# lambdaclass/noir_backend_using_gnark

Hardware: AMD Instinct MI355X
Metric: Groth16 prove ms + BN254 G1 MSM scalar-muls/sec at 2^20 / 2^24 constraints (higher is better)
Workload: dtype u32

## Files before the change

### noir_backend_using_gnark_amd/csrc/groth16.hip

```cpp
#include <stdlib.h>
#include <chrono>
#include <functional>
#include <memory>
#include <vector>
#include <string.h>

#include "ctx.hpp"
#include "curve.hpp"
#include "host_ff.hpp"
#include "keyio.hpp"
#include "msm.hpp"
#include "multidev.hpp"
#include "ntt.hpp"
#include "proofio.hpp"

namespace zkmi {

template <class F>
struct FixedBase {
    std::vector<XYZZ<F>> tab;
    void build(const Affine<F>& p) {
        tab.resize(32 * 256);
        XYZZ<F> base = XYZZ<F>::from_affine(p);
        for (int w = 0; w < 32; w++) {
// ... 320 lines not shown
    auto it = g_pks.find(handle);
    if (it == g_pks.end()) return set_err(ZK_ERR_HANDLE, "unknown proving-key handle %llu", (unsigned long long)handle);
    if (n_wires) *n_wires = it->second.n_wires;
    if (n_public) *n_public = it->second.n_public;
    if (log_domain) *log_domain = it->second.log_domain;
    if (has_tables) *has_tables = it->second.tables ? 1 : 0;
    return ZK_OK;
}

struct Msm5Inputs {
    const void *d_a, *d_b, *d_b2, *d_w;
    size_t nw;
    const void *d_k, *d_wk;
    size_t nk;
    const void *d_z, *d_h;
    size_t nz;
    const MsmTable *tab_w = nullptr, *tab_h = nullptr;
    const void *t_a = nullptr, *t_b = nullptr, *t_b2 = nullptr, *t_k = nullptr, *t_z = nullptr;
};
static const zk_msm_cfg kMontCfg = {0, 1, 0, 0};

static bool k_shares_w(const Msm5Inputs& in, size_t* j) {
    if (!in.nk || !in.nw) return false;
    ptrdiff_t d = (const char*)in.d_wk - (const char*)in.d_w;
    if (d < 0 || d % 32) return false;
    *j = (size_t)d / 32;
    return *j + in.nk == in.nw;
}

struct Msm5State {
    MsmJob jobs[5];
    MsmPrep prep_w, prep_h;
    hipStream_t chain = nullptr;
};

static int msm5_prepare_w(Slot* sl[5], const Msm5Inputs& in, hipEvent_t ev_w, Msm5State* S) {
    static const bool low = ZK_EXP("ZKMI_PREPW_LOW", 0) == 1;
    hipStream_t st4 = low ? sl[4]->stream : sl[4]->hi();
    if (ev_w) ZK_HIP(hipStreamWaitEvent(st4, ev_w, 0));
    static const bool drop = ZK_EXP("ZKMI_W_DROP_ZERO_DIGITS", 1) != 0;
    if (in.tab_w) return msm_prepare_scalars_table(sl[4], st4, in.d_w, in.nw, &kMontCfg, *in.tab_w, &S->prep_w, drop);
    return msm_prepare_scalars(sl[4], st4, in.d_w, in.nw, &kMontCfg, &S->prep_w, drop);
}
typedef std::function<int(hipEvent_t g2_done, hipEvent_t* gate_next)> BetweenFn;
static int msm5_accumulate_w(Slot* sl[5], const Msm5Inputs& in, hipEvent_t ev_w, Msm5State* S, hipEvent_t gate_first_acc, const BetweenFn* between = nullptr);
static int msm5_launch_w(Slot* sl[5], const Msm5Inputs& in, hipEvent_t ev_w, Msm5State* S, hipEvent_t gate_first_acc = nullptr) {
    ZK_TRY(msm5_prepare_w(sl, in, ev_w, S));
    return msm5_accumulate_w(sl, in, ev_w, S, gate_first_acc);
}
static int msm5_accumulate_w(Slot* sl[5], const Msm5Inputs& in, hipEvent_t ev_w, Msm5State* S, hipEvent_t gate_first_acc, const BetweenFn* between) {
    hipStream_t st4 = sl[4]->hi();
    size_t j = 0;
    const bool share_k = k_shares_w(in, &j);
    static const bool one_chain = ZK_EXP("ZKMI_CHAIN", 0) == 1;
    if (one_chain && (in.tab_w || share_k)) {
        hipStream_t chain = sl[4]->stream;
        S->jobs[4].gate_acc = gate_first_acc;
        S->jobs[4].chain = chain;
        ZK_TRY(msm_g2_accumulate(sl[4], st4, S->prep_w, in.tab_w ? in.t_b2 : in.d_b2, 0, &S->jobs[4]));
        S->jobs[1].chain = chain;
        ZK_TRY(msm_g1_accumulate(sl[1], sl[1]->stream, S->prep_w, in.tab_w ? in.t_a : in.d_a, 0, &S->jobs[1]));
        S->jobs[2].chain = chain;
        ZK_TRY(msm_g1_accumulate(sl[2], sl[2]->stream, S->prep_w, in.tab_w ? in.t_b : in.d_b, 0, &S->jobs[2]));
        S->jobs[3].chain = chain;
        S->jobs[3].want_done = true;
        if (in.tab_w) ZK_TRY(msm_g1_accumulate(sl[3], sl[3]->stream, S->prep_w, in.t_k, 0, &S->jobs[3]));
        else ZK_TRY(msm_g1_accumulate(sl[3], sl[3]->stream, S->prep_w, (const char*)in.d_k - j * 64, (uint32_t)j, &S->jobs[3]));
        return ZK_OK;
    }
    S->jobs[4].gate_acc = gate_first_acc;
    S->jobs[4].want_done = true;
    ZK_TRY(msm_g2_accumulate(sl[4], st4, S->prep_w, in.tab_w ? in.t_b2 : in.d_b2, 0, &S->jobs[4]));
    hipEvent_t prev = S->jobs[4].acc_done;
    if (between) ZK_TRY((*between)(S->jobs[4].acc_done, &prev));
    static const bool batch_acc = ZK_EXP("ZKMI_BATCH_ACC", 0) == 1;
    if (batch_acc && (in.tab_w || share_k)) {
        Slot* bs[3] = {sl[1], sl[2], sl[3]};
        hipStream_t bst[3] = {sl[1]->stream, sl[2]->stream, sl[3]->stream};
        const void* bp[3] = {in.tab_w ? in.t_a : in.d_a, in.tab_w ? in.t_b : in.d_b, in.tab_w ? in.t_k : (const void*)((const char*)in.d_k - j * 64)};
        uint32_t bskip[3] = {0, 0, in.tab_w ? 0u : (uint32_t)j};
        MsmJob* bj[3] = {&S->jobs[1], &S->jobs[2], &S->jobs[3]};
        S->jobs[1].gate_acc = prev;
        S->jobs[3].want_done = true;
        return msm_g1_accumulate_batch(3, bs, bst, S->prep_w, bp, bskip, bj);
    }
    S->jobs[1].gate_acc = prev;
    S->jobs[1].want_done = true;
    ZK_TRY(msm_g1_accumulate(sl[1], sl[1]->stream, S->prep_w, in.tab_w ? in.t_a : in.d_a, 0, &S->jobs[1]));
    if (S->jobs[1].acc_done) prev = S->jobs[1].acc_done;
    S->jobs[2].gate_acc = prev;
    S->jobs[2].want_done = true;
    ZK_TRY(msm_g1_accumulate(sl[2], sl[2]->stream, S->prep_w, in.tab_w ? in.t_b : in.d_b, 0, &S->jobs[2]));
    if (S->jobs[2].acc_done) prev = S->jobs[2].acc_done;
    S->jobs[3].gate_acc = prev;
    S->jobs[3].want_done = true;
    if (in.tab_w) {
        ZK_TRY(msm_g1_accumulate(sl[3], sl[3]->stream, S->prep_w, in.t_k, 0, &S->jobs[3]));
    } else if (share_k) {
        ZK_TRY(msm_g1_accumulate(sl[3], sl[3]->stream, S->prep_w, (const char*)in.d_k - j * 64, (uint32_t)j, &S->jobs[3]));
    } else {
        if (ev_w) ZK_HIP(hipStreamWaitEvent(sl[3]->stream, ev_w, 0));
        ZK_TRY(msm_g1_launch(sl[3], sl[3]->stream, in.d_k, in.d_wk, in.nk, &kMontCfg, &S->jobs[3]));
    }
    return ZK_OK;
}
static int msm5_prepare_h(Slot* sl[5], hipStream_t st0, const Msm5Inputs& in, Msm5State* S) {
    if (in.tab_h) return msm_prepare_scalars_table(sl[0], st0, in.d_h, in.nz, &kMontCfg, *in.tab_h, &S->prep_h);
    return msm_prepare_scalars(sl[0], st0, in.d_h, in.nz, &kMontCfg, &S->prep_h);
}
static int msm5_launch_h(Slot* sl[5], hipStream_t st0, const Msm5Inputs& in, Msm5State* S, bool prepared = false) {
    static const bool preph_low = ZK_EXP("ZKMI_PREPH_LOW", 0) == 1;
    if (!prepared && preph_low && sl[0]->stream != st0) {
        hipEvent_t ev;
        ZK_HIP(hipEventCreateWithFlags(&ev, hipEventDisableTiming));
        ZK_HIP(hipEventRecord(ev, st0));
        ZK_HIP(hipStreamWaitEvent(sl[0]->stream, ev, 0));
        (void)hipEventDestroy(ev);
        ZK_TRY(msm5_prepare_h(sl, sl[0]->stream, in, S));
        prepared = true;
    }
    if (!prepared) ZK_TRY(msm5_prepare_h(sl, st0, in, S));
    S->jobs[0].chain = S->chain;
    if (!S->chain) {
        hipEvent_t prev = nullptr;
        for (int i : {4, 1, 2, 3})
            if (S->jobs[i].acc_done) prev = S->jobs[i].acc_done;
        S->jobs[0].gate_acc = prev;
    }
    static const bool quad_tail = ZK_EXP("ZKMI_QUAD_TAIL", 0) == 1;
    S->jobs[0].quad_tail = quad_tail;
    ZK_TRY(msm_g1_accumulate(sl[0], st0, S->prep_h, in.tab_h ? in.t_z : in.d_z, 0, &S->jobs[0]));
    return ZK_OK;
}
static int msm5_finish(Msm5State* S, uint64_t out[96], const std::function<void(const XYZZ<HFp>&, const XYZZ<HFp>&)>* early = nullptr) {
    XYZZ<HFp> m_a, m_b, m_k, m_z;
    XYZZ<HFp2> m_b2;
    int rc = msm_g2_finish(S->jobs[4], &m_b2);
    if (rc == ZK_OK) rc = msm_g1_finish(S->jobs[1], &m_a);
    if (rc == ZK_OK) rc = msm_g1_finish(S->jobs[2], &m_b);
    if (rc == ZK_OK && early) (*early)(m_a, m_b);
    if (rc == ZK_OK) rc = msm_g1_finish(S->jobs[3], &m_k);
    if (rc == ZK_OK) rc = msm_g1_finish(S->jobs[0], &m_z);
    msm_prep_release(&S->prep_w);
    msm_prep_release(&S->prep_h);
    for (int i = 0; i < 5; i++)
        if (S->jobs[i].acc_done) { (void)hipEventDestroy(S->jobs[i].acc_done); S->jobs[i].acc_done = nullptr; }
    ZK_TRY(rc);
    memcpy(out, &m_a, 128);
    memcpy(out + 16, &m_b, 128);
    memcpy(out + 32, &m_k, 128);
    memcpy(out + 48, &m_z, 128);
    memcpy(out + 64, &m_b2, 256);
    return ZK_OK;
}
static int msm5_reserve(Slot* sl[5], const Msm5Inputs& in, size_t extra0) {
    size_t need[5] = {0, 0, 0, 0, 0}, prep = 0, acc1 = 0, acc2 = 0, j = 0;
    if (in.tab_h) {
        size_t ph = 0, ah = 0;
        ZK_TRY(msm_prep_need_table(in.nz, *in.tab_h, sl[0]->stream, &ph, &ah, nullptr));
        need[0] = ph + ah;
    } else {
        ZK_TRY(msm_g1_need(in.nz, &kMontCfg, sl[0]->stream, &need[0]));
    }
// ... 290 lines not shown
        in.t_a = P.t_a; in.t_b = P.t_b; in.t_b2 = P.t_b2; in.t_k = P.t_k; in.t_z = P.t_z;
    }
    ZK_TRY(msm5_reserve(g.s, in, 3 * N * 32 + nw * 32 + 4096));
    hipMemcpyKind kind = on_device ? hipMemcpyDeviceToDevice : hipMemcpyHostToDevice;
    hipStream_t st4 = g.s[4]->hi();
    int rc = ZK_OK;
    Fr* d_abc[3] = {nullptr, nullptr, nullptr};
    const void* src[3] = {a, b, c};
    const bool direct = on_device && n_constraints == N && N > 1;
    static const bool host_order_on = (ZK_EXP("ZKMI_HOST_ORDER", 1) != 0);
    const bool host_order = !on_device && host_order_on && nw > 0 && N > 1;
    Fr* d_w = (Fr*)s0->alloc(nw * 32 + 16);
    for (int i = 0; i < 3; i++) d_abc[i] = (Fr*)s0->alloc(N * 32);
    if (on_device) d_w = (Fr*)const_cast<void*>(w);
    auto upload_abc = [&]() -> int {
        for (int i = 0; i < 3; i++) {
            if (direct) continue;
            if (n_constraints && hipMemcpyAsync(d_abc[i], src[i], n_constraints * 32, kind, st) != hipSuccess) return set_err(ZK_ERR_HIP, "hipMemcpyAsync failed");
            if (n_constraints < N && hipMemsetAsync(d_abc[i] + n_constraints, 0, (N - n_constraints) * 32, st) != hipSuccess) return set_err(ZK_ERR_HIP, "hipMemsetAsync failed");
        }
        return ZK_OK;
    };
    const Fr* in_place_src[3] = {(const Fr*)a, (const Fr*)b, (const Fr*)c};
    static const bool h_streams = ZK_EXP("ZKMI_H_STREAMS", 0) == 1;
    const hipStream_t side[2] = {g.s[1]->hi(), g.s[2]->hi()};
    hipEvent_t ev_h = nullptr;
    auto run_compute_h = [&]() -> int {
        ZK_TRY(compute_h_inplace(s0, st, d_abc[0], d_abc[1], d_abc[2], P.log_domain, direct ? in_place_src : nullptr, h_streams ? side : nullptr));
        ZK_HIP(hipEventCreateWithFlags(&ev_h, hipEventDisableTiming));
        ZK_HIP(hipEventRecord(ev_h, st));
        return ZK_OK;
    };
    Msm5State S;
    static const bool nogate = ZK_EXP("ZKMI_NOGATE", 0) == 1;
    static const bool preph_first = ZK_EXP("ZKMI_PREPH_FIRST", 0) == 1;
    static const bool preph_early = ZK_EXP("ZKMI_PREPH_EARLY", 0) == 1;
    if (host_order) {
        if (hipMemcpyAsync(d_w, w, nw * 32, kind, st4) != hipSuccess) rc = set_err(ZK_ERR_HIP, "hipMemcpyAsync failed");
        in.d_w = d_w;
        in.d_wk = d_w + P.n_public;
        in.d_h = d_abc[0];
        if (rc == ZK_OK) rc = msm5_prepare_w(g.s, in, nullptr, &S);
        if (rc == ZK_OK) rc = upload_abc();
        const BetweenFn between = [&](hipEvent_t g2_done, hipEvent_t* gate_next) -> int {
            if (g2_done) ZK_HIP(hipStreamWaitEvent(st, g2_done, 0));
            ZK_TRY(run_compute_h());
            *gate_next = ev_h;
            return ZK_OK;
        };
        if (rc == ZK_OK) rc = msm5_accumulate_w(g.s, in, nullptr, &S, nullptr, &between);
        if (rc == ZK_OK) rc = msm5_launch_h(g.s, st, in, &S);
    } else {
        static const bool h_under_g2 = ZK_EXP("ZKMI_H_UNDER_G2", 0) == 1;
        if (h_under_g2) {
            if (!on_device && nw && hipMemcpyAsync(d_w, w, nw * 32, kind, st4) != hipSuccess) rc = set_err(ZK_ERR_HIP, "hipMemcpyAsync failed");
            in.d_w = d_w;
            in.d_wk = d_w + P.n_public;
            in.d_h = d_abc[0];
            if (rc == ZK_OK) rc = msm5_prepare_w(g.s, in, nullptr, &S);
            if (rc == ZK_OK) rc = upload_abc();
            if (rc == ZK_OK && S.prep_w.ready && hipStreamWaitEvent(st, S.prep_w.ready, 0) != hipSuccess) rc = set_err(ZK_ERR_HIP, "hipStreamWaitEvent failed");
            if (rc == ZK_OK) rc = run_compute_h();
            if (rc == ZK_OK) rc = msm5_accumulate_w(g.s, in, nullptr, &S, nullptr);
            if (rc == ZK_OK) rc = msm5_launch_h(g.s, st, in, &S);
        } else {
        rc = upload_abc();
// ... 39 lines not shown
```

### noir_backend_using_gnark_amd/csrc/msm.hip

```cpp
#include <math.h>
#include <string.h>

#include <algorithm>
#include <memory>
#include <tuple>
#include <type_traits>

#ifdef ZKMI_EXPERIMENTS
#include "experiments/msm_rocprim_include.inc"
#endif

#include <chrono>
#include "ctx.hpp"
#include "curve.hpp"
#include "ff29.hpp"
#include "host_ff.hpp"
#include "msm.hpp"
#include "multidev.hpp"
#include "radix.hpp"

namespace zkmi {

struct PingPong {
    uint32_t* b[2];
// ... 685 lines not shown
            for (uint32_t t = t0 + lane; t < t1; t += 64) acc.add(TailPt<F>::load(partial + t));
        }
        const uint32_t cnt = min(nheld, 64u);
        unsigned first = 32;
        while (first >= cnt && first > 0) first >>= 1;
        for (unsigned d = first; d > 0; d >>= 1) {
            TailPt<F> o = acc.shfl_down(d);
            if (lane < d) acc.add(o);
        }
        if (lane == 0) acc.store(partial + t0);
    }
}

template <class F, class PT = TailPt<F>>
__global__ __launch_bounds__(256) void k_reduce_l1(const XYZZ<F>* __restrict__ partial, const uint32_t* __restrict__ task_off, uint32_t B,
                                                   uint32_t W, uint32_t m, XYZZ<F>* __restrict__ A_out, XYZZ<F>* __restrict__ S_out) {
    prio_hi();
    uint32_t N1 = B / m;
    uint32_t g = (blockIdx.x * blockDim.x + threadIdx.x) / PT::LPP;
    if (g >= W * N1) return;
    uint32_t w = g / N1, q = g % N1;
    uint32_t b0 = w * B + q * m;
    PT run = PT::inf(), acc = PT::inf();
    for (int l = (int)m - 1; l >= 0; l--) {
        uint32_t b = b0 + l;
        uint32_t t0 = task_off[b];
        if (task_off[b + 1] > t0) run.add(PT::load(partial + t0));
        acc.add(run);
    }
    if (threadIdx.x % PT::LPP == 0) {
        acc.store(A_out + g);
        run.store(S_out + g);
    }
}

template <class F>
__global__ __launch_bounds__(256) void k_reduce_l2(const XYZZ<F>* __restrict__ A_in, const XYZZ<F>* __restrict__ S_in, uint32_t N, uint32_t W, uint32_t sh,
                                                   uint32_t m, XYZZ<F>* __restrict__ A_out, XYZZ<F>* __restrict__ S_out) {
    prio_hi();
    typedef TailPt<F> PT;
    uint32_t Nout = (N + m - 1) / m;
    uint32_t g = blockIdx.x * blockDim.x + threadIdx.x;
    if (g >= W * Nout) return;
    uint32_t w = g / Nout, q = g % Nout;
    PT run = PT::inf(), t = PT::inf(), asum = PT::inf();
    for (int l = (int)m - 1; l >= 0; l--) {
        uint32_t j = q * m + (uint32_t)l;
        if (j >= N) continue;
        asum.add(PT::load(A_in + (size_t)w * N + j));
        run.add(PT::load(S_in + (size_t)w * N + j));
        if (l >= 1) t.add(run);
    }
    for (uint32_t i = 0; i < sh; i++) t.dbl();
    asum.add(t);
    asum.store(A_out + g);
    run.store(S_out + g);
}

template <class F, class PT = TailPt<F>>
__global__ __launch_bounds__(64) void k_reduce_wave(const XYZZ<F>* __restrict__ A_in, const XYZZ<F>* __restrict__ S_in, uint32_t N, uint32_t W,
                                                    uint32_t sh, XYZZ<F>* __restrict__ A_out, XYZZ<F>* __restrict__ S_out) {
    prio_hi();
    constexpr uint32_t FAN = 64 / PT::LPP;
    uint32_t Nout = (N + FAN - 1) / FAN;
    uint32_t chunk = blockIdx.x;
    uint32_t w = chunk / Nout, q = chunk % Nout;
// ... 226 lines not shown
#include "experiments/msm_scan_rocprim_call.inc"
#endif
    if (own_scan) ZK_TRY(xs_exclusive_scan(s, st, scan_tmp, ntasks, task_off, (size_t)nb + 1));
    }
    uint32_t bshift = 0;
    while ((L >> bshift) >= TS_BINS) bshift++;
    const uint32_t nbins = (L >> bshift) + 1;
    const unsigned tgrid = (unsigned)((max_tasks + 255) / 256);
    static const bool merged_fill = ZK_EXP("ZKMI_PREP_MERGE", 1) == 2;
    if (merged_fill) {
        ZK_LAUNCH(s, st, "msm_task_fill", k_task_fill_bins, dim3(tgrid), dim3(256), 0, (const uint32_t*)start, (const uint32_t*)task_off, nb, L, bins, (uint32_t)max_tasks, bshift,
                  nbins, task_begin, lkey0, hist);
    } else {
        ZK_LAUNCH(s, st, "msm_task_fill", k_task_fill, dim3(tgrid), dim3(256), 0, (const uint32_t*)start, (const uint32_t*)task_off, nb, L, (const uint32_t*)bins,
                  (uint32_t)max_tasks, bshift, nbins, task_begin, lkey0, hist);
        ZK_LAUNCH(s, st, "msm_task_bins", k_task_bins, dim3(1), dim3(256), 0, hist, nbins);
    }
    ZK_LAUNCH(s, st, "msm_task_scatter", k_task_scatter, dim3(tgrid), dim3(256), 0, (const uint32_t*)lkey0, (uint32_t)max_tasks, bshift, nbins, hist,
              lkey1, tid1);
    out->vals = vb.current();
    out->start = start;
    out->task_off = task_off;
    out->task_begin = task_begin;
    out->lkeys = lkey1;
    out->tids = tid1;
    out->multi_list = multi_list;
    out->num_multi = num_multi;
    ZK_HIP(hipEventCreateWithFlags(&out->ready, hipEventDisableTiming));
    ZK_HIP(hipEventRecord(out->ready, st));
    return ZK_OK;
}

template <class F>
static int msm_accumulate_batch(int nb, Slot* const* sl, const hipStream_t* sts, const MsmPrep& R, const void* const* d_pts, const uint32_t* skip_below,
                                MsmJob* const* jobs) {
    typedef XYZZ<F> Pt;
    const MsmPlan& P = R.P;
    for (int b = 0; b < nb; b++) {
        jobs[b]->s = sl[b];
        jobs[b]->st = sts[b];
        jobs[b]->c = P.c;
        jobs[b]->W = P.W;
        jobs[b]->empty = R.empty;
    }
    if (R.empty) return ZK_OK;
    const unsigned W = P.W;
    const uint32_t B = P.B, L = P.L, m1 = P.m1, N1 = P.N1;
    const size_t max_tasks = P.max_tasks, lvl_elems = P.lvl_elems;
    Pt *partial[3], *lvlA[3][2], *lvlS[3][2];
    AccBatch batch = {};
    for (int b = 0; b < nb; b++) {
        Slot* s = sl[b];
        partial[b] = (Pt*)s->alloc(max_tasks * sizeof(Pt));
        for (int k = 0; k < 2; k++) {
            lvlA[b][k] = (Pt*)s->alloc((lvl_elems + 64) * sizeof(Pt));
            lvlS[b][k] = (Pt*)s->alloc((lvl_elems + 64) * sizeof(Pt));
        }
        if (!partial[b] || !lvlA[b][0] || !lvlA[b][1] || !lvlS[b][0] || !lvlS[b][1])
            return set_err(ZK_ERR_HIP, "MSM workspace was not reserved up front (%zu bytes needed)", P.need_acc);
        batch.pts[b] = d_pts[b];
        batch.partial[b] = partial[b];
        batch.skip_below[b] = skip_below[b];
    }
    MsmJob* j0 = jobs[0];
    hipStream_t sa = j0->chain ? j0->chain : sts[0];
    if (R.ready) ZK_HIP(hipStreamWaitEvent(sa, R.ready, 0));
// ... 39 lines not shown
        }
    }
#endif
    if (!launched) ZK_LAUNCH(sl[0], sa, acc_name, (k_accumulate<F>), dim3(full_grid, (unsigned)nb), dim3(256), acc_shmem, batch, R.vals, R.task_begin, R.lkeys, R.tids, L, (uint32_t)max_tasks);
    if (T) {
        hipEvent_t& e = T->ring[T->next];
        if (!e) ZK_HIP(hipEventCreateWithFlags(&e, hipEventDisableTiming));
        ZK_HIP(hipEventRecord(e, sa));
        T->last = e;
        T->next = (T->next + 1) % 16;
        turn_lock.unlock();
    }
    bool want = j0->chain != nullptr || nb > 1;
    for (int b = 0; b < nb; b++) want = want || jobs[b]->want_done;
    if (want) {
        hipEvent_t done;
        ZK_HIP(hipEventCreateWithFlags(&done, hipEventDisableTiming));
        ZK_HIP(hipEventRecord(done, sa));
        jobs[nb - 1]->acc_done = done;
        for (int b = 0; b < nb; b++)
            if (sts[b] != sa) ZK_HIP(hipStreamWaitEvent(sts[b], done, 0));
    }
    for (int b = 0; b < nb; b++) {
        Slot* s = sl[b];
        hipStream_t st = sts[b];
        bool folded = false;
#ifdef ZKMI_EXPERIMENTS
#include "experiments/msm_tail_fused_launch.inc"
#endif
        if (!folded) {
            ZK_LAUNCH(s, st, "msm_fold_giant", (k_fold_giant<F>), dim3(GIANT_MAX * 16), dim3(256), 0, partial[b], R.task_off, (const uint32_t*)R.num_multi);
            ZK_LAUNCH(s, st, "msm_fold_multi", (k_fold_multi<F>), dim3(1024), dim3(256), 0, partial[b], R.task_off, R.multi_list, R.num_multi);
        }
        bool quad = false;
        if constexpr (sizeof(F) == sizeof(Fp)) quad = jobs[b]->quad_tail;
        const uint32_t lpp = quad ? 4 : 1, fan = 64 / lpp, fan_log = quad ? 4 : 6;
        ZK_LAUNCH(s, st, "msm_reduce_l1", (k_reduce_l1<F>), dim3((unsigned)(((size_t)W * N1 + 255) / 256)), dim3(256), 0, (const Pt*)partial[b], R.task_off, B, W,
                  m1, lvlA[b][0], lvlS[b][0]);
        uint32_t N = N1, sh = 0;
        for (uint32_t mm = m1; mm > 1; mm >>= 1) sh++;
        int cur = 0;
        if (P.m2 > 1 && N > 64 * P.m2) {
            uint32_t Nout = (N + P.m2 - 1) / P.m2;
            ZK_LAUNCH(s, st, "msm_reduce_l2", (k_reduce_l2<F>), dim3((unsigned)(((size_t)W * Nout + 255) / 256)), dim3(256), 0, (const Pt*)lvlA[b][cur],
                      (const Pt*)lvlS[b][cur], N, W, sh, P.m2, lvlA[b][cur ^ 1], lvlS[b][cur ^ 1]);
            cur ^= 1;
            N = Nout;
            for (uint32_t mm = P.m2; mm > 1; mm >>= 1) sh++;
        }
        const uint32_t host_n = (W * 64 <= 64) ? 64 : 1;
        while (N > host_n) {
            uint32_t Nout = (N + fan - 1) / fan;
            if constexpr (sizeof(F) == sizeof(Fp)) {
                if (quad) ZK_LAUNCH(s, st, "msm_reduce_wave", (k_reduce_wave<F, TailPtQ>), dim3(W * Nout), dim3(64), 0, (const Pt*)lvlA[b][cur], (const Pt*)lvlS[b][cur], N, W, sh, lvlA[b][cur ^ 1], lvlS[b][cur ^ 1]);
            }
            if (!quad) ZK_LAUNCH(s, st, "msm_reduce_wave", (k_reduce_wave<F>), dim3(W * Nout), dim3(64), 0, (const Pt*)lvlA[b][cur], (const Pt*)lvlS[b][cur], N, W, sh, lvlA[b][cur ^ 1], lvlS[b][cur ^ 1]);
            cur ^= 1;
            N = Nout;
            sh += fan_log;
        }
        jobs[b]->n_final = N;
        jobs[b]->sh_final = sh;
        const size_t cnt = (size_t)W * N;
        ZK_TRY(s->pinned_reserve(2 * cnt * sizeof(Pt)));
        ZK_HIP(hipMemcpyAsync(s->pinned, lvlA[b][cur], cnt * sizeof(Pt), hipMemcpyDeviceToHost, st));
        if (N > 1) ZK_HIP(hipMemcpyAsync((char*)s->pinned + cnt * sizeof(Pt), lvlS[b][cur], cnt * sizeof(Pt), hipMemcpyDeviceToHost, st));
    }
    return ZK_OK;
}

template <class F>
static int msm_accumulate(Slot* s, hipStream_t st, const MsmPrep& R, const Affine<F>* d_pts, uint32_t skip_below, MsmJob* job) {
    const void* pts = d_pts;
    return msm_accumulate_batch<F>(1, &s, &st, R, &pts, &skip_below, &job);
}

template <class F>
static int msm_launch(Slot* s, hipStream_t st, const MsmPlan& P, const Affine<F>* d_pts, const Fr* d_scalars, size_t n, const zk_msm_cfg* cfg,
                      MsmJob* job) {
    MsmPrep R;
    ZK_TRY(msm_prepare(s, st, P, d_scalars, n, cfg, &R));
    int rc = msm_accumulate<F>(s, st, R, d_pts, 0, job);
    if (R.ready) (void)hipEventDestroy(R.ready);
    return rc;
}

template <class HF>
static int msm_finish(const MsmJob& job, XYZZ<HF>* total_out, XYZZ<HF>* per_set = nullptr) {
    *total_out = XYZZ<HF>::inf();
    if (per_set)
        for (unsigned w = 0; w < (job.empty ? 3u : job.W); w++) per_set[w] = XYZZ<HF>::inf();
    if (job.empty) return ZK_OK;
    ZK_TRY(slot_sync(job.s, job.st));
    const unsigned N = job.n_final;
    if constexpr (sizeof(HF) == sizeof(HFp)) {
        static const HFp inv32 = HFp{{32, 0, 0, 0}}.to_mont().inv();
        XYZZ<HFp>* w = reinterpret_cast<XYZZ<HFp>*>(job.s->pinned);
        const size_t cnt = (size_t)job.W * N * (N > 1 ? 2 : 1);
        for (size_t i = 0; i < cnt; i++) {
            w[i].x = w[i].x * inv32;
            w[i].y = w[i].y * inv32;
            w[i].zz = w[i].zz * inv32;
            w[i].zzz = w[i].zzz * inv32;
        }
    }
    const XYZZ<HF>* wa = reinterpret_cast<const XYZZ<HF>*>(job.s->pinned);
    const XYZZ<HF>* wsum = wa + (size_t)job.W * N;
// ... 176 lines not shown
    uint32_t j = src_idx[i];
    Affine<F> p;
    uint4* d = reinterpret_cast<uint4*>(&p);
    if (j == 0xffffffffu) {
#pragma unroll
        for (unsigned k = 0; k < sizeof(p) / 16; k++) d[k] = make_uint4(0, 0, 0, 0);
    } else {
        p = gload(compact + j);
    }
    gstore(out + i, p);
}
int msm_expand_bases(Slot* s, hipStream_t st, int is_g2, const void* d_compact, const uint32_t* d_src_idx, size_t n, void* d_out) {
    if (!n) return ZK_OK;
    if (is_g2)
        ZK_LAUNCH(s, st, "pk_expand_bases_g2", (k_expand_bases<Fp2>), dim3((unsigned)((n + 255) / 256)), dim3(256), 0, (const Affine<Fp2>*)d_compact, d_src_idx,
                  (uint32_t)n, (Affine<Fp2>*)d_out);
    else
        ZK_LAUNCH(s, st, "pk_expand_bases_g1", (k_expand_bases<Fp>), dim3((unsigned)((n + 255) / 256)), dim3(256), 0, (const Affine<Fp>*)d_compact, d_src_idx,
                  (uint32_t)n, (Affine<Fp>*)d_out);
    return ZK_OK;
}

int msm_prepare_scalars(Slot* s, hipStream_t st, const void* d_scalars, size_t n, const zk_msm_cfg* cfg, MsmPrep* out, bool drop_zero_digits) {
    MsmPlan P;
    ZK_TRY(msm_plan<Fp>(n, cfg, st, &P));
    return msm_prepare(s, st, P, (const Fr*)d_scalars, n, cfg, out, nullptr, drop_zero_digits);
}
void msm_prep_release(MsmPrep* R) {
    if (R->ready) (void)hipEventDestroy(R->ready);
    R->ready = nullptr;
}
int msm_g1_accumulate(Slot* s, hipStream_t st, const MsmPrep& R, const void* d_pts, uint32_t skip_below, MsmJob* job) {
    return msm_accumulate<Fp>(s, st, R, (const Affine<Fp>*)d_pts, skip_below, job);
}
int msm_g1_accumulate_batch(int nb, Slot* const* sl, const hipStream_t* sts, const MsmPrep& R, const void* const* d_pts, const uint32_t* skip_below,
                            MsmJob* const* jobs) {
    if (nb < 1 || nb > 3) return set_err(ZK_ERR_ARG, "accumulate batch of %d", nb);
    return msm_accumulate_batch<Fp>(nb, sl, sts, R, d_pts, skip_below, jobs);
}
int msm_g2_accumulate(Slot* s, hipStream_t st, const MsmPrep& R, const void* d_pts, uint32_t skip_below, MsmJob* job) {
    return msm_accumulate<Fp2>(s, st, R, (const Affine<Fp2>*)d_pts, skip_below, job);
}
int msm_g1_finish(const MsmJob& job, XYZZ<HFp>* out) { return msm_finish<HFp>(job, out); }
int msm_g1_finish_batch(const MsmJob& job, XYZZ<HFp> out[3]) {
    XYZZ<HFp> unused;
    return msm_finish<HFp>(job, &unused, out);
}
int msm_g2_finish(const MsmJob& job, XYZZ<HFp2>* out) { return msm_finish<HFp2>(job, out); }
int msm_g1_xyzz(Slot* s, hipStream_t st, const void* d_pts, const void* d_scalars, size_t n, const zk_msm_cfg* cfg, XYZZ<HFp>* out) {
    MsmJob job;
    ZK_TRY(msm_g1_launch(s, st, d_pts, d_scalars, n, cfg, &job));
    return msm_g1_finish(job, out);
}
int msm_g2_xyzz(Slot* s, hipStream_t st, const void* d_pts, const void* d_scalars, size_t n, const zk_msm_cfg* cfg, XYZZ<HFp2>* out) {
    MsmJob job;
    ZK_TRY(msm_g2_launch(s, st, d_pts, d_scalars, n, cfg, &job));
    return msm_g2_finish(job, out);
}

static int check_cfg(const zk_msm_cfg* cfg) {
    if (cfg && cfg->nb_tasks > 1024) return set_err(ZK_ERR_NB_TASKS, "invalid config: config.NbTasks > 1024");
    return ZK_OK;
}

struct Bases {
    void* d = nullptr;
// ... 569 lines not shown
```

### noir_backend_using_gnark_amd/csrc/msm.hpp

```cpp
#pragma once
#include "ctx.hpp"
#include "curve.hpp"
#include "host_ff.hpp"

namespace zkmi {

unsigned msm_pick_window(size_t n);
int msm_g1_need(size_t n, const zk_msm_cfg* cfg, hipStream_t st, size_t* need);
int msm_g2_need(size_t n, const zk_msm_cfg* cfg, hipStream_t st, size_t* need);
struct MsmTable {
    unsigned c = 0;
    size_t stride = 0;
    unsigned row_first = 0, row_step = 1;
    unsigned rows() const {
        unsigned Wd = (255 + c - 1) / c;
        return row_first < Wd ? (Wd - 1 - row_first) / row_step + 1 : 0;
    }
    unsigned l2_m = 0;
    unsigned l1_m = 0;
};
unsigned msm_pick_window_table(size_t n);
int msm_build_table_g1(Slot* s, hipStream_t st, const void* d_pts, size_t n, size_t stride, size_t offset, unsigned c, void* d_table, unsigned row_first = 0,
                       unsigned row_step = 1);
int msm_build_table_g2(Slot* s, hipStream_t st, const void* d_pts, size_t n, size_t stride, size_t offset, unsigned c, void* d_table, unsigned row_first = 0,
// ... 22 lines not shown
    hipEvent_t ready = nullptr;
};

struct MsmJob {
    Slot* s = nullptr;
    hipStream_t st = nullptr;
    unsigned c = 0, W = 0;
    unsigned n_final = 1, sh_final = 0;
    bool empty = true;
    hipEvent_t gate_acc = nullptr;
    bool want_done = false;
    hipEvent_t acc_done = nullptr;
    hipStream_t chain = nullptr;
    bool turnstile = false;
    bool quad_tail = false;
};
int msm_g1_launch(Slot* s, hipStream_t st, const void* d_pts, const void* d_scalars, size_t n, const zk_msm_cfg* cfg, MsmJob* job);
int msm_g2_launch(Slot* s, hipStream_t st, const void* d_pts, const void* d_scalars, size_t n, const zk_msm_cfg* cfg, MsmJob* job);
int msm_prep_need(size_t n, const zk_msm_cfg* cfg, hipStream_t st, size_t* need_prep, size_t* need_acc_g1, size_t* need_acc_g2);
int msm_prepare_scalars(Slot* s, hipStream_t st, const void* d_scalars, size_t n, const zk_msm_cfg* cfg, MsmPrep* out, bool drop_zero_digits = false);
int msm_prep_need_table(size_t n, const MsmTable& tab, hipStream_t st, size_t* need_prep, size_t* need_acc_g1, size_t* need_acc_g2);
int msm_prepare_scalars_table(Slot* s, hipStream_t st, const void* d_scalars, size_t n, const zk_msm_cfg* cfg, const MsmTable& tab, MsmPrep* out, bool drop_zero_digits = false);
int msm_prep_need_table_batch(size_t n, unsigned sets, const MsmTable& tab, hipStream_t st, size_t* need_prep, size_t* need_acc_g1);
int msm_prepare_scalars_table_batch(Slot* s, hipStream_t st, const void* const* d_scalars, unsigned sets, size_t n, const zk_msm_cfg* cfg, const MsmTable& tab, MsmPrep* out,
                                    bool drop_zero_digits = false);
size_t msm_compact_need(size_t n, unsigned sets);
int msm_bases_batch_dev_sparse(uint64_t handle, size_t offset, const void* const* d_scalars, unsigned count, size_t n, const zk_msm_cfg* cfg, void* out);
int msm_g1_finish_batch(const MsmJob& job, XYZZ<HFp> out[3]);
void msm_prep_release(MsmPrep* R);
int msm_g1_accumulate(Slot* s, hipStream_t st, const MsmPrep& R, const void* d_pts, uint32_t skip_below, MsmJob* job);
int msm_g2_accumulate(Slot* s, hipStream_t st, const MsmPrep& R, const void* d_pts, uint32_t skip_below, MsmJob* job);
int msm_g1_accumulate_batch(int nb, Slot* const* sl, const hipStream_t* sts, const MsmPrep& R, const void* const* d_pts, const uint32_t* skip_below,
                            MsmJob* const* jobs);
int msm_g1_finish(const MsmJob& job, XYZZ<HFp>* out);
int msm_g2_finish(const MsmJob& job, XYZZ<HFp2>* out);
int msm_g1_xyzz(Slot* s, hipStream_t st, const void* d_pts, const void* d_scalars, size_t n, const zk_msm_cfg* cfg, XYZZ<HFp>* out);
int msm_g2_xyzz(Slot* s, hipStream_t st, const void* d_pts, const void* d_scalars, size_t n, const zk_msm_cfg* cfg, XYZZ<HFp2>* out);

}
```

Measured before the change: 449.6 million.

## Merge K and H MSMs into one shared bucket reduction tail

When the witness K MSM and the H/Z MSM use the same bucket layout, both are still accumulated into their own per-task partials. A new pair kernel then sums the two bucket sets inside a single level-1 reduction, so only one reduction chain and one host finish run instead of two. The reduction code is moved into a shared helper to support this. It adds cross-stream event dependencies and skips the separate K job, which relies on the finish step treating that job as empty.

```diff
diff --git a/noir_backend_using_gnark_amd/csrc/groth16.hip b/noir_backend_using_gnark_amd/csrc/groth16.hip
--- a/noir_backend_using_gnark_amd/csrc/groth16.hip
+++ b/noir_backend_using_gnark_amd/csrc/groth16.hip
@@ -376,7 +376,18 @@
     MsmJob jobs[5];
     MsmPrep prep_w, prep_h;
     hipStream_t chain = nullptr;
+    bool kz_allowed = false, kz = false;
 };
+
+static bool kz_merge(const Msm5Inputs& in, hipStream_t st) {
+    static const bool on = ZK_EXP("ZKMI_KZ_MERGE", 1) != 0;
+    size_t j = 0;
+    if (!on || !in.nw || !in.nk || !in.nz || (in.tab_w == nullptr) != (in.tab_h == nullptr)) return false;
+    if (in.tab_w && (in.tab_w->row_step > 1 || in.tab_h->row_step > 1)) return false;
+    if (!in.tab_w && !k_shares_w(in, &j)) return false;
+    bool ok = false;
+    return msm_g1_pair_ok(in.nw, in.tab_w, in.nz, in.tab_h, &kMontCfg, st, &ok) == ZK_OK && ok;
+}
 
 static int msm5_prepare_w(Slot* sl[5], const Msm5Inputs& in, hipEvent_t ev_w, Msm5State* S) {
     static const bool low = ZK_EXP("ZKMI_PREPW_LOW", 0) == 1;
@@ -396,8 +407,10 @@
     hipStream_t st4 = sl[4]->hi();
     size_t j = 0;
     const bool share_k = k_shares_w(in, &j);
+    S->kz = S->kz_allowed && kz_merge(in, st4);
     static const bool one_chain = ZK_EXP("ZKMI_CHAIN", 0) == 1;
     if (one_chain && (in.tab_w || share_k)) {
+        S->kz = false;
         hipStream_t chain = sl[4]->stream;
         S->jobs[4].gate_acc = gate_first_acc;
         S->jobs[4].chain = chain;
@@ -419,6 +432,7 @@
     if (between) ZK_TRY((*between)(S->jobs[4].acc_done, &prev));
     static const bool batch_acc = ZK_EXP("ZKMI_BATCH_ACC", 0) == 1;
     if (batch_acc && (in.tab_w || share_k)) {
+        S->kz = false;
         Slot* bs[3] = {sl[1], sl[2], sl[3]};
         hipStream_t bst[3] = {sl[1]->stream, sl[2]->stream, sl[3]->stream};
         const void* bp[3] = {in.tab_w ? in.t_a : in.d_a, in.tab_w ? in.t_b : in.d_b, in.tab_w ? in.t_k : (const void*)((const char*)in.d_k - j * 64)};
@@ -435,6 +449,7 @@
     S->jobs[2].gate_acc = prev;
     S->jobs[2].want_done = true;
     ZK_TRY(msm_g1_accumulate(sl[2], sl[2]->stream, S->prep_w, in.tab_w ? in.t_b : in.d_b, 0, &S->jobs[2]));
+    if (S->kz) return ZK_OK;
     if (S->jobs[2].acc_done) prev = S->jobs[2].acc_done;
     S->jobs[3].gate_acc = prev;
     S->jobs[3].want_done = true;
@@ -473,6 +488,16 @@
     }
     static const bool quad_tail = ZK_EXP("ZKMI_QUAD_TAIL", 0) == 1;
     S->jobs[0].quad_tail = quad_tail;
+    if (S->kz) {
+        size_t j = 0;
+        const bool share_k = !in.tab_w && k_shares_w(in, &j);
+        Slot* const psl[2] = {sl[3], sl[0]};
+        const hipStream_t psts[2] = {sl[3]->stream, st0};
+        const MsmPrep* const pR[2] = {&S->prep_w, &S->prep_h};
+        const void* const ppts[2] = {in.tab_w ? in.t_k : (const void*)((const char*)in.d_k - j * 64), in.tab_h ? in.t_z : in.d_z};
+        const uint32_t pskip[2] = {share_k ? (uint32_t)j : 0u, 0u};
+        return msm_g1_accumulate_pair(psl, psts, pR, ppts, pskip, &S->jobs[0]);
+    }
     ZK_TRY(msm_g1_accumulate(sl[0], st0, S->prep_h, in.tab_h ? in.t_z : in.d_z, 0, &S->jobs[0]));
     return ZK_OK;
 }
@@ -829,6 +854,7 @@
         return ZK_OK;
     };
     Msm5State S;
+    S.kz_allowed = true;
     static const bool nogate = ZK_EXP("ZKMI_NOGATE", 0) == 1;
     static const bool preph_first = ZK_EXP("ZKMI_PREPH_FIRST", 0) == 1;
     static const bool preph_early = ZK_EXP("ZKMI_PREPH_EARLY", 0) == 1;
diff --git a/noir_backend_using_gnark_amd/csrc/msm.hip b/noir_backend_using_gnark_amd/csrc/msm.hip
--- a/noir_backend_using_gnark_amd/csrc/msm.hip
+++ b/noir_backend_using_gnark_amd/csrc/msm.hip
@@ -741,6 +741,28 @@
         acc.store(A_out + g);
         run.store(S_out + g);
     }
+}
+template <class F>
+__global__ __launch_bounds__(256) void k_reduce_l1_pair(const XYZZ<F>* __restrict__ partial0, const uint32_t* __restrict__ task_off0,
+                                                        const XYZZ<F>* __restrict__ partial1, const uint32_t* __restrict__ task_off1, uint32_t B, uint32_t W,
+                                                        uint32_t m, XYZZ<F>* __restrict__ A_out, XYZZ<F>* __restrict__ S_out) {
+    prio_hi();
+    typedef TailPt<F> PT;
+    uint32_t N1 = B / m;
+    uint32_t g = blockIdx.x * blockDim.x + threadIdx.x;
+    if (g >= W * N1) return;
+    uint32_t w = g / N1, q = g % N1;
+    uint32_t b0 = w * B + q * m;
+    PT run = PT::inf(), acc = PT::inf();
+    for (int l = (int)m - 1; l >= 0; l--) {
+        uint32_t b = b0 + l;
+        uint32_t t0 = task_off0[b], t1 = task_off1[b];
+        if (task_off0[b + 1] > t0) run.add(PT::load(partial0 + t0));
+        if (task_off1[b + 1] > t1) run.add(PT::load(partial1 + t1));
+        acc.add(run);
+    }
+    acc.store(A_out + g);
+    run.store(S_out + g);
 }
 
 template <class F>
@@ -1033,6 +1055,44 @@
 }
 
 template <class F>
+static int msm_reduce_levels(Slot* s, hipStream_t st, const MsmPlan& P, XYZZ<F>* const lvlA[2], XYZZ<F>* const lvlS[2], MsmJob* job) {
+    typedef XYZZ<F> Pt;
+    const unsigned W = P.W;
+    bool quad = false;
+    if constexpr (sizeof(F) == sizeof(Fp)) quad = job->quad_tail;
+    const uint32_t lpp = quad ? 4 : 1, fan = 64 / lpp, fan_log = quad ? 4 : 6;
+    uint32_t N = P.N1, sh = 0;
+    for (uint32_t mm = P.m1; mm > 1; mm >>= 1) sh++;
+    int cur = 0;
+    if (P.m2 > 1 && N > 64 * P.m2) {
+        uint32_t Nout = (N + P.m2 - 1) / P.m2;
+        ZK_LAUNCH(s, st, "msm_reduce_l2", (k_reduce_l2<F>), dim3((unsigned)(((size_t)W * Nout + 255) / 256)), dim3(256), 0, (const Pt*)lvlA[cur],
+                  (const Pt*)lvlS[cur], N, W, sh, P.m2, lvlA[cur ^ 1], lvlS[cur ^ 1]);
+        cur ^= 1;
+        N = Nout;
+        for (uint32_t mm = P.m2; mm > 1; mm >>= 1) sh++;
+    }
+    const uint32_t host_n = (W * 64 <= 64) ? 64 : 1;
+    while (N > host_n) {
+        uint32_t Nout = (N + fan - 1) / fan;
+        if constexpr (sizeof(F) == sizeof(Fp)) {
+            if (quad) ZK_LAUNCH(s, st, "msm_reduce_wave", (k_reduce_wave<F, TailPtQ>), dim3(W * Nout), dim3(64), 0, (const Pt*)lvlA[cur], (const Pt*)lvlS[cur], N, W, sh, lvlA[cur ^ 1], lvlS[cur ^ 1]);
+        }
+        if (!quad) ZK_LAUNCH(s, st, "msm_reduce_wave", (k_reduce_wave<F>), dim3(W * Nout), dim3(64), 0, (const Pt*)lvlA[cur], (const Pt*)lvlS[cur], N, W, sh, lvlA[cur ^ 1], lvlS[cur ^ 1]);
+        cur ^= 1;
+        N = Nout;
+        sh += fan_log;
+    }
+    job->n_final = N;
+    job->sh_final = sh;
+    const size_t cnt = (size_t)W * N;
+    ZK_TRY(s->pinned_reserve(2 * cnt * sizeof(Pt)));
+    ZK_HIP(hipMemcpyAsync(s->pinned, lvlA[cur], cnt * sizeof(Pt), hipMemcpyDeviceToHost, st));
+    if (N > 1) ZK_HIP(hipMemcpyAsync((char*)s->pinned + cnt * sizeof(Pt), lvlS[cur], cnt * sizeof(Pt), hipMemcpyDeviceToHost, st));
+    return ZK_OK;
+}
+
+template <class F>
 static int msm_accumulate_batch(int nb, Slot* const* sl, const hipStream_t* sts, const MsmPrep& R, const void* const* d_pts, const uint32_t* skip_below,
                                 MsmJob* const* jobs) {
     typedef XYZZ<F> Pt;
@@ -1138,39 +1198,9 @@
             ZK_LAUNCH(s, st, "msm_fold_giant", (k_fold_giant<F>), dim3(GIANT_MAX * 16), dim3(256), 0, partial[b], R.task_off, (const uint32_t*)R.num_multi);
             ZK_LAUNCH(s, st, "msm_fold_multi", (k_fold_multi<F>), dim3(1024), dim3(256), 0, partial[b], R.task_off, R.multi_list, R.num_multi);
         }
-        bool quad = false;
-        if constexpr (sizeof(F) == sizeof(Fp)) quad = jobs[b]->quad_tail;
-        const uint32_t lpp = quad ? 4 : 1, fan = 64 / lpp, fan_log = quad ? 4 : 6;
         ZK_LAUNCH(s, st, "msm_reduce_l1", (k_reduce_l1<F>), dim3((unsigned)(((size_t)W * N1 + 255) / 256)), dim3(256), 0, (const Pt*)partial[b], R.task_off, B, W,
                   m1, lvlA[b][0], lvlS[b][0]);
-        uint32_t N = N1, sh = 0;
-        for (uint32_t mm = m1; mm > 1; mm >>= 1) sh++;
-        int cur = 0;
-        if (P.m2 > 1 && N > 64 * P.m2) {
-            uint32_t Nout = (N + P.m2 - 1) / P.m2;
-            ZK_LAUNCH(s, st, "msm_reduce_l2", (k_reduce_l2<F>), dim3((unsigned)(((size_t)W * Nout + 255) / 256)), dim3(256), 0, (const Pt*)lvlA[b][cur],
-                      (const Pt*)lvlS[b][cur], N, W, sh, P.m2, lvlA[b][cur ^ 1], lvlS[b][cur ^ 1]);
-            cur ^= 1;
-            N = Nout;
-            for (uint32_t mm = P.m2; mm > 1; mm >>= 1) sh++;
-        }
-        const uint32_t host_n = (W * 64 <= 64) ? 64 : 1;
-        while (N > host_n) {
-            uint32_t Nout = (N + fan - 1) / fan;
-            if constexpr (sizeof(F) == sizeof(Fp)) {
-                if (quad) ZK_LAUNCH(s, st, "msm_reduce_wave", (k_reduce_wave<F, TailPtQ>), dim3(W * Nout), dim3(64), 0, (const Pt*)lvlA[b][cur], (const Pt*)lvlS[b][cur], N, W, sh, lvlA[b][cur ^ 1], lvlS[b][cur ^ 1]);
-            }
-            if (!quad) ZK_LAUNCH(s, st, "msm_reduce_wave", (k_reduce_wave<F>), dim3(W * Nout), dim3(64), 0, (const Pt*)lvlA[b][cur], (const Pt*)lvlS[b][cur], N, W, sh, lvlA[b][cur ^ 1], lvlS[b][cur ^ 1]);
-            cur ^= 1;
-            N = Nout;
-            sh += fan_log;
-        }
-        jobs[b]->n_final = N;
-        jobs[b]->sh_final = sh;
-        const size_t cnt = (size_t)W * N;
-        ZK_TRY(s->pinned_reserve(2 * cnt * sizeof(Pt)));
-        ZK_HIP(hipMemcpyAsync(s->pinned, lvlA[b][cur], cnt * sizeof(Pt), hipMemcpyDeviceToHost, st));
-        if (N > 1) ZK_HIP(hipMemcpyAsync((char*)s->pinned + cnt * sizeof(Pt), lvlS[b][cur], cnt * sizeof(Pt), hipMemcpyDeviceToHost, st));
+        ZK_TRY(msm_reduce_levels<F>(s, st, P, lvlA[b], lvlS[b], jobs[b]));
     }
     return ZK_OK;
 }
@@ -1179,6 +1209,64 @@
 static int msm_accumulate(Slot* s, hipStream_t st, const MsmPrep& R, const Affine<F>* d_pts, uint32_t skip_below, MsmJob* job) {
     const void* pts = d_pts;
     return msm_accumulate_batch<F>(1, &s, &st, R, &pts, &skip_below, &job);
+}
+
+static bool plans_pair(const MsmPlan& a, const MsmPlan& b) {
+    return a.c == b.c && a.W == b.W && a.B == b.B && a.nb == b.nb && a.Wrows == b.Wrows && a.row_first == b.row_first && a.row_step == b.row_step;
+}
+static int msm_g1_accumulate_pair_impl(Slot* const sl[2], const hipStream_t sts[2], const MsmPrep* const R[2], const void* const d_pts[2], const uint32_t skip_below[2],
+                                       MsmJob* job) {
+    typedef XYZZ<Fp> Pt;
+    const MsmPlan& P = R[1]->P;
+    if (R[0]->empty || R[1]->empty || !plans_pair(R[0]->P, P)) return set_err(ZK_ERR_ARG, "the two preparations do not share one bucket layout");
+    job->s = sl[1];
+    job->st = sts[1];
+    job->c = P.c;
+    job->W = P.W;
+    job->empty = false;
+    Pt* partial[2];
+    for (int k = 0; k < 2; k++) {
+        partial[k] = (Pt*)sl[k]->alloc(R[k]->P.max_tasks * sizeof(Pt));
+        if (!partial[k]) return set_err(ZK_ERR_HIP, "MSM workspace was not reserved up front (%zu bytes needed)", R[k]->P.need_acc);
+    }
+    Pt *lvlA[2], *lvlS[2];
+    for (int k = 0; k < 2; k++) {
+        lvlA[k] = (Pt*)sl[1]->alloc((P.lvl_elems + 64) * sizeof(Pt));
+        lvlS[k] = (Pt*)sl[1]->alloc((P.lvl_elems + 64) * sizeof(Pt));
+        if (!lvlA[k] || !lvlS[k]) return set_err(ZK_ERR_HIP, "MSM workspace was not reserved up front (%zu bytes needed)", P.need_acc);
+    }
+    hipEvent_t ev[2] = {nullptr, nullptr};
+    auto destroy = [&]() { for (hipEvent_t e : ev) if (e) (void)hipEventDestroy(e); };
+    int rc = ZK_OK;
+    auto step = [&](hipError_t e) { if (rc == ZK_OK && e != hipSuccess) rc = set_err(ZK_ERR_HIP, "%s", hipGetErrorString(e)); };
+    for (hipEvent_t& e : ev) step(hipEventCreateWithFlags(&e, hipEventDisableTiming));
+    for (int k = 0; k < 2 && rc == ZK_OK; k++) {
+        if (R[k]->ready) step(hipStreamWaitEvent(sts[k], R[k]->ready, 0));
+        if (k == 0 && job->gate_acc) step(hipStreamWaitEvent(sts[0], job->gate_acc, 0));
+        if (k == 1) step(hipStreamWaitEvent(sts[1], ev[0], 0));
+        if (rc != ZK_OK) break;
+        AccBatch batch = {};
+        batch.pts[0] = d_pts[k];
+        batch.partial[0] = partial[k];
+        batch.skip_below[0] = skip_below[k];
+        const MsmPlan& Pk = R[k]->P;
+        ZK_LAUNCH(sl[k], sts[k], "msm_accumulate_g1", (k_accumulate<Fp>), dim3((unsigned)((Pk.max_tasks + 255) / 256), 1u), dim3(256), 0, batch, R[k]->vals,
+                  R[k]->task_begin, R[k]->lkeys, R[k]->tids, Pk.L, (uint32_t)Pk.max_tasks);
+        if (k == 0) step(hipEventRecord(ev[0], sts[0]));
+        if (k == 1 && job->want_done) {
+            step(hipEventCreateWithFlags(&job->acc_done, hipEventDisableTiming));
+            step(hipEventRecord(job->acc_done, sts[1]));
+        }
+        ZK_LAUNCH(sl[k], sts[k], "msm_fold_giant", (k_fold_giant<Fp>), dim3(GIANT_MAX * 16), dim3(256), 0, partial[k], R[k]->task_off, (const uint32_t*)R[k]->num_multi);
+        ZK_LAUNCH(sl[k], sts[k], "msm_fold_multi", (k_fold_multi<Fp>), dim3(1024), dim3(256), 0, partial[k], R[k]->task_off, R[k]->multi_list, R[k]->num_multi);
+        if (k == 0) step(hipEventRecord(ev[1], sts[0]));
+    }
+    if (rc == ZK_OK) step(hipStreamWaitEvent(sts[1], ev[1], 0));
+    destroy();
+    ZK_TRY(rc);
+    ZK_LAUNCH(sl[1], sts[1], "msm_reduce_l1_pair", k_reduce_l1_pair<Fp>, dim3((unsigned)(((size_t)P.W * P.N1 + 255) / 256)), dim3(256), 0, (const Pt*)partial[0], R[0]->task_off,
+              (const Pt*)partial[1], R[1]->task_off, P.B, P.W, P.m1, lvlA[0], lvlS[0]);
+    return msm_reduce_levels<Fp>(sl[1], sts[1], P, lvlA, lvlS, job);
 }
 
 template <class F>
@@ -1421,6 +1509,18 @@
 }
 int msm_g1_accumulate(Slot* s, hipStream_t st, const MsmPrep& R, const void* d_pts, uint32_t skip_below, MsmJob* job) {
     return msm_accumulate<Fp>(s, st, R, (const Affine<Fp>*)d_pts, skip_below, job);
+}
+int msm_g1_pair_ok(size_t n0, const MsmTable* t0, size_t n1, const MsmTable* t1, const zk_msm_cfg* cfg, hipStream_t st, bool* ok) {
+    *ok = false;
+    if (!n0 || !n1 || (t0 == nullptr) != (t1 == nullptr)) return ZK_OK;
+    MsmPlan P0, P1;
+    ZK_TRY(msm_plan<Fp>(n0, t0 ? nullptr : cfg, st, &P0, t0));
+    ZK_TRY(msm_plan<Fp>(n1, t1 ? nullptr : cfg, st, &P1, t1));
+    *ok = P0.total && P1.total && plans_pair(P0, P1);
+    return ZK_OK;
+}
+int msm_g1_accumulate_pair(Slot* const sl[2], const hipStream_t sts[2], const MsmPrep* const R[2], const void* const d_pts[2], const uint32_t skip_below[2], MsmJob* job) {
+    return msm_g1_accumulate_pair_impl(sl, sts, R, d_pts, skip_below, job);
 }
 int msm_g1_accumulate_batch(int nb, Slot* const* sl, const hipStream_t* sts, const MsmPrep& R, const void* const* d_pts, const uint32_t* skip_below,
                             MsmJob* const* jobs) {
diff --git a/noir_backend_using_gnark_amd/csrc/msm.hpp b/noir_backend_using_gnark_amd/csrc/msm.hpp
--- a/noir_backend_using_gnark_amd/csrc/msm.hpp
+++ b/noir_backend_using_gnark_amd/csrc/msm.hpp
@@ -78,6 +78,8 @@
 int msm_g2_accumulate(Slot* s, hipStream_t st, const MsmPrep& R, const void* d_pts, uint32_t skip_below, MsmJob* job);
 int msm_g1_accumulate_batch(int nb, Slot* const* sl, const hipStream_t* sts, const MsmPrep& R, const void* const* d_pts, const uint32_t* skip_below,
                             MsmJob* const* jobs);
+int msm_g1_pair_ok(size_t n0, const MsmTable* t0, size_t n1, const MsmTable* t1, const zk_msm_cfg* cfg, hipStream_t st, bool* ok);
+int msm_g1_accumulate_pair(Slot* const sl[2], const hipStream_t sts[2], const MsmPrep* const R[2], const void* const d_pts[2], const uint32_t skip_below[2], MsmJob* job);
 int msm_g1_finish(const MsmJob& job, XYZZ<HFp>* out);
 int msm_g2_finish(const MsmJob& job, XYZZ<HFp2>* out);
 int msm_g1_xyzz(Slot* s, hipStream_t st, const void* d_pts, const void* d_scalars, size_t n, const zk_msm_cfg* cfg, XYZZ<HFp>* out);
```

Result: faster. 456.8 million (median of 6 runs) (+1.6%).
